# onesamblack/distributed-torch-horovod-gcp

Measured on NVIDIA H100. Metric: images/sec (whole job, device-timed, max over ranks) ResNet-50 synthetic ImageNet training, higher is better.
Workload: dtype bf16

## Files before the change

### distributed_torch_horovod_gcp_b200/csrc/conv_sm90.cu

```cuda
#include <cuda.h>
#include <cuda_bf16.h>
#include <cuda_runtime.h>
#include <limits.h>
#include <stdint.h>
#include <stdio.h>
#include <stdlib.h>
#include <string.h>

#include "sm90_common.cuh"

namespace {

constexpr int MAX_TAPS = 9;
constexpr int MAX_CLASSES = 4;

struct ConvTap {
  int amap;
  int dw, dh;
  int wcol;
};
struct ConvClass {
  int ntaps;
  int out_map;
  ConvTap taps[MAX_TAPS];
// ... 61 lines not shown
          } else {
#pragma unroll
            for (int c = 0; c < BN / 64; ++c)
              tma_load_2d(&maps.b, s.bar, s.b + c * (BLOCK_K * 128), tap.wcol + n_idx + 64 * c, kc * BLOCK_K);
          }
        }
      }
    } else {
      const int tile = w % tiles, split = w / tiles;
      const ConvTap tap = p.cls[0].taps[tile % p.num_taps_total];
      const int mn = tile / p.num_taps_total;
      const int m_idx = (mn / nnb) * BLOCK_M;
      const int n_idx = (mn % nnb) * BN;
      const int kb0 = split * kb_per_split;
      const int kb1 = min(kb0 + kb_per_split, pix_tiles);
      for (int kb = kb0; kb < kb1; ++kb) {
        const int w0 = (kb % p.tiles_w) * p.bw;
        const int h0 = ((kb / p.tiles_w) % p.tiles_h) * p.bh;
        const int n0 = (kb / (p.tiles_w * p.tiles_h)) * p.bn;
        const Stage s = next();
#pragma unroll
        for (int c = 0; c < BLOCK_M / 64; ++c)
          tma_load_4d(&maps.out[0], s.bar, s.a + c * (BLOCK_K * 128), m_idx + 64 * c, w0, h0, n0);
#pragma unroll
        for (int c = 0; c < BN / 64; ++c)
          tma_load_4d(&maps.a[tap.amap], s.bar, s.b + c * (BLOCK_K * 128), n_idx + 64 * c, w0 + tap.dw,
                      h0 + tap.dh, n0);
      }
    }
  }
  __device__ Slab slab(int w, int q) const {
    if (MODE != MODE_WGRAD) {
      const int nt = w % nnb;
      const int rest = w / nnb;
      const int mt = rest % pix_tiles;
      const int r0 = q * 32;
      StoreAt at;
      at.rank4 = 1;
      at.w = (mt % p.tiles_w) * p.bw + (r0 % p.bw);
      at.h = ((mt / p.tiles_w) % p.tiles_h) * p.bh + (r0 / p.bw) % p.bh;
      at.n = (mt / (p.tiles_w * p.tiles_h)) * p.bn + r0 / (p.bw * p.bh);
      at.sw = p.sw; at.sh = p.sh;
      at.vw = p.out_w - at.w; at.vh = p.out_h - at.h; at.vn = p.out_n - at.n;
      return Slab{&maps.out[p.cls[rest / pix_tiles].out_map], 0, nt * BN, at, 0, 0, 0, 0};
    }
    const int tile = w % tiles;
    const ConvTap tap = p.cls[0].taps[tile % p.num_taps_total];
    const int mn = tile / p.num_taps_total;
    const int m_idx = (mn / nnb) * BLOCK_M;
    return Slab{nullptr, m_idx + q * 32, (mn % nnb) * BN, StoreAt{}, tile, m_idx, tap.wcol, w / tiles};
  }
};

template <int BN, int MODE>
__global__ void __launch_bounds__(NUM_THREADS, 1)
conv_bf16_kernel(const __grid_constant__ ConvMaps maps, const __grid_constant__ ConvParams p) {
  persistent_body<BN, MODE == MODE_WGRAD, MODE != MODE_FPROP>(ConvWork<BN, MODE>(maps, p), p.g);
}

int make_map4(CUtensorMap* m, const void* ptr, uint64_t C, uint64_t Wd, uint64_t Hd, uint64_t Nd, uint64_t pw,
              uint64_t ph, uint64_t pn, uint32_t bw, uint32_t bh, uint32_t bn) {
  const cuuint64_t dims[4] = {C, Wd, Hd, Nd};
  const cuuint64_t strides[3] = {pw * 2, ph * 2, pn * 2};
  const cuuint32_t box[4] = {64, bw, bh, bn};
  return encode_map(m, ptr, 4, dims, strides, box);
}

void choose_box(int W, int H, int N, int rows, int* bw, int* bh, int* bn) {
  double best = 1e30;
  *bw = 1; *bh = 1; *bn = rows;
  for (int w = 1; w <= rows; w <<= 1) {
    for (int h = 1; w * h <= rows; h <<= 1) {
      const int n = rows / (w * h);
      const double covered = (double)((W + w - 1) / w * w) * ((H + h - 1) / h * h) * ((N + n - 1) / n * n);
      const double score = covered - 1e-3 * w - 1e-6 * h;
      if (score < best) { best = score; *bw = w; *bh = h; *bn = n; }
    }
  }
}

int floordiv2(int e) { return (e >= 0) ? e / 2 : -((-e + 1) / 2); }

struct ConvShape {
  int N, H, W, Cin, Cout, R, S, stride, pad, OH, OW;
};

int check_shape(ConvShape& s) {
  if (s.R != s.S || (s.R != 1 && s.R != 3)) return fail("only 1x1 and 3x3 filters");
  if (s.pad != (s.R - 1) / 2) return fail("padding must be (R-1)/2");
  if (s.stride != 1 && s.stride != 2) return fail("stride must be 1 or 2");
  if (s.stride == 2 && ((s.H | s.W) & 1)) return fail("stride 2 needs even H and W");
  if ((s.Cin % 8) || (s.Cout % 8)) return fail("channels must be multiples of 8");
  s.OH = s.H / s.stride;
  s.OW = s.W / s.stride;
  return 0;
}

int make_parity_maps(CUtensorMap* maps, const void* base, int C, int W, int H, int N, int bw, int bh, int bn) {
  for (int ph = 0; ph < 2; ++ph)
    for (int pw = 0; pw < 2; ++pw) {
      const __nv_bfloat16* ptr = reinterpret_cast<const __nv_bfloat16*>(base) + ((size_t)ph * W + pw) * C;
      if (make_map4(&maps[ph * 2 + pw], ptr, C, W / 2, H / 2, N, 2 * (uint64_t)C, 2 * (uint64_t)W * C,
                    (uint64_t)H * W * C, bw, bh, bn))
        return -1;
    }
  return 0;
}

void forward_taps(ConvClass& cl, int R, int S, int Cin, int stride, int pad) {
  for (int r = 0; r < R; ++r)
    for (int c = 0; c < S; ++c) {
      ConvTap& t = cl.taps[cl.ntaps++];
      const int eh = r - pad, ew = c - pad;
      if (stride == 1) {
        t.amap = 0; t.dh = eh; t.dw = ew;
      } else {
        const int ph = eh & 1, pw = ew & 1;
        t.amap = ph * 2 + pw; t.dh = floordiv2(eh - ph); t.dw = floordiv2(ew - pw);
      }
      t.wcol = (r * S + c) * Cin;
    }
}

void slab_box(ConvParams& p) {
  p.sw = p.bw < 32 ? p.bw : 32;
  p.sh = (32 / p.sw) < p.bh ? (32 / p.sw) : p.bh;
}

template <int MODE>
int launch_conv(const ConvMaps& maps, const ConvParams& p, int BN, int work, int max_ctas, cudaStream_t st) {
  if (BN == 64) return launch_persistent<conv_bf16_kernel<64, MODE>, 64>(work, max_ctas, st, maps, p);
  return launch_persistent<conv_bf16_kernel<128, MODE>, 128>(work, max_ctas, st, maps, p);
}

ConvParams conv_params() {
  ConvParams p;
  memset(&p, 0, sizeof(p));
  p.g.M = INT_MAX;
  p.g.splits = 1;
  p.g.alpha = 1.0f;
  return p;
}

}

extern "C" {

const char* b200dp_conv_last_error() { return g_err; }

int b200dp_conv_fprop(const void* x, const void* w, void* y, int N, int H, int W, int Cin, int Cout, int R, int S,
                      int stride, int pad, int block_n, int max_ctas, float* stats, unsigned long long stream) {
  if (ensure_init()) return -1;
  ConvShape s{N, H, W, Cin, Cout, R, S, stride, pad, 0, 0};
  if (check_shape(s)) return -1;
  if (((uintptr_t)x | (uintptr_t)w | (uintptr_t)y) & 15) return fail("pointers must be 16-byte aligned");
  const int BN = pick_bn(Cout, block_n);
  if (BN < 0) return -1;
  ConvMaps maps;
  ConvParams p = conv_params();
  p.g.N = Cout; p.g.ldc = Cout; p.g.C = y; p.g.out_mode = 0;
  p.g.stats = stats;
  if (stats != nullptr && Cout > STATS_MAX_N) return fail("stats: Cout <= 2048 required");
  p.g.num_n_blocks = (Cout + BN - 1) / BN;
  p.g.num_k_blocks = (Cin + BLOCK_K - 1) / BLOCK_K;
  p.kc_per_tap = p.g.num_k_blocks;
  choose_box(s.OW, s.OH, N, BLOCK_M, &p.bw, &p.bh, &p.bn);
  p.tiles_w = (s.OW + p.bw - 1) / p.bw; p.tiles_h = (s.OH + p.bh - 1) / p.bh; p.tiles_n = (N + p.bn - 1) / p.bn;
  p.num_classes = 1;
  p.num_taps_total = R * S;
  p.out_w = s.OW; p.out_h = s.OH; p.out_n = N;
  forward_taps(p.cls[0], R, S, Cin, stride, pad);
  if (stride == 1) {
    if (make_map4(&maps.a[0], x, Cin, W, H, N, Cin, (uint64_t)W * Cin, (uint64_t)H * W * Cin, p.bw, p.bh, p.bn))
      return -1;
    maps.a[1] = maps.a[2] = maps.a[3] = maps.a[0];
  } else if (make_parity_maps(maps.a, x, Cin, W, H, N, p.bw, p.bh, p.bn)) {
    return -1;
  }
  if (make_map2(&maps.b, w, Cout, (uint64_t)R * S * Cin, (uint64_t)R * S * Cin, BN)) return -1;
  slab_box(p);
  if (make_map4(&maps.out[0], y, Cout, s.OW, s.OH, N, Cout, (uint64_t)s.OW * Cout, (uint64_t)s.OH * s.OW * Cout, p.sw,
                p.sh, 32 / (p.sw * p.sh)))
    return -1;
  maps.out[1] = maps.out[2] = maps.out[3] = maps.out[0];
  const int work = p.tiles_w * p.tiles_h * p.tiles_n * p.g.num_n_blocks;
// ... 119 lines not shown
```

### distributed_torch_horovod_gcp_b200/csrc/gemm_sm90.cu

```cuda
#include <cuda.h>
#include <cuda_bf16.h>
#include <cuda_runtime.h>
#include <stdint.h>

#include "sm90_common.cuh"

namespace {

template <int BN, bool A_MN, bool B_MN>
struct GemmWork {
  static constexpr bool kStats = true, kSplitK = true;
  const CUtensorMap *a, *b, *c;
  const GemmParams& p;
  int tiles, items, kb_per_split;

  __device__ GemmWork(const CUtensorMap* a_, const CUtensorMap* b_, const CUtensorMap* c_, const GemmParams& p_)
      : a(a_), b(b_), c(c_), p(p_), tiles(p_.num_m_blocks * p_.num_n_blocks), items(tiles * p_.splits),
        kb_per_split((p_.num_k_blocks + p_.splits - 1) / p_.splits) {}
  __device__ void prefetch() const {
    tma_prefetch_desc(a);
    tma_prefetch_desc(b);
    if (p.out_mode == 0) tma_prefetch_desc(c);
  }
  __device__ int m_idx(int tile) const {
    return (p.n_fastest ? tile / p.num_n_blocks : tile % p.num_m_blocks) * BLOCK_M;
  }
  __device__ int n_idx(int tile) const { return (p.n_fastest ? tile % p.num_n_blocks : tile / p.num_m_blocks) * BN; }
  __device__ int num_kb(int w) const {
    const int kb0 = (w / tiles) * kb_per_split;
    return min(kb0 + kb_per_split, p.num_k_blocks) - kb0;
  }
  template <class Next>
  __device__ void load(int w, Next& next) const {
    const int tile = w % tiles;
    const int m0 = m_idx(tile), n0 = n_idx(tile);
    const int kb0 = (w / tiles) * kb_per_split;
    const int kb1 = min(kb0 + kb_per_split, p.num_k_blocks);
    for (int kb = kb0; kb < kb1; ++kb) {
      const Stage s = next();
      const int k_idx = kb * BLOCK_K;
      if (!A_MN) {
        tma_load_2d(a, s.bar, s.a, k_idx, m0);
      } else {
#pragma unroll
        for (int c = 0; c < BLOCK_M / 64; ++c)
          tma_load_2d(a, s.bar, s.a + c * (BLOCK_K * 128), m0 + 64 * c, k_idx);
      }
      if (!B_MN) {
        tma_load_2d(b, s.bar, s.b, k_idx, n0);
      } else {
#pragma unroll
        for (int c = 0; c < BN / 64; ++c)
          tma_load_2d(b, s.bar, s.b + c * (BLOCK_K * 128), n0 + 64 * c, k_idx);
      }
    }
  }
  __device__ Slab slab(int w, int q) const {
    const int tile = w % tiles, split = w / tiles;
    const int m0 = m_idx(tile);
    return Slab{c, m0 + q * 32, n_idx(tile), StoreAt{}, tile, m0, 0, split};
  }
};

template <int BN, bool A_MN, bool B_MN>
__global__ void __launch_bounds__(NUM_THREADS, 1)
gemm_bf16_kernel(const __grid_constant__ CUtensorMap map_a, const __grid_constant__ CUtensorMap map_b,
                 const __grid_constant__ CUtensorMap map_c, const __grid_constant__ GemmParams p) {
  persistent_body<BN, A_MN, B_MN>(GemmWork<BN, A_MN, B_MN>(&map_a, &map_b, &map_c, p), p);
}

int launch_bn(int BN, int a_mn, int b_mn, const CUtensorMap& ma, const CUtensorMap& mb, const CUtensorMap& mc,
              const GemmParams& p, int max_ctas, cudaStream_t st) {
  const int work = p.num_m_blocks * p.num_n_blocks * p.splits;
#define LAUNCH(BNV, AMN, BMN) \
  launch_persistent<gemm_bf16_kernel<BNV, AMN, BMN>, BNV>(work, max_ctas, st, ma, mb, mc, p)
#define DISPATCH(BNV)                                          \
  if (BN == BNV) {                                             \
    if (!a_mn && !b_mn) return LAUNCH(BNV, false, false);      \
    if (!a_mn && b_mn) return LAUNCH(BNV, false, true);        \
    if (a_mn && !b_mn) return LAUNCH(BNV, true, false);        \
    return LAUNCH(BNV, true, true);                            \
  }
  DISPATCH(64)
  DISPATCH(128)
#undef DISPATCH
#undef LAUNCH
  return fail("unreachable");
}

}

extern "C" {

const char* b200dp_gemm_last_error() { return g_err; }

int b200dp_gemm_bf16(const void* A, const void* B, void* C, int M, int N, int K, int lda, int ldb, int ldc,
                     int a_mn, int b_mn, const void* bias_bf16, const void* bias_f32, const void* residual,
                     void* preact, int act, int out_mode, int out_bf16, float alpha, int splits, int block_n,
                     int max_ctas, float* stats, const void* res_mask, unsigned long long stream) {
  if (ensure_init()) return -1;
  if (M <= 0 || N <= 0 || K <= 0) return fail("bad shape");
  if ((N % 8) || (lda % 8) || (ldb % 8) || (ldc % 4) || ((out_mode == 0 || out_bf16) && (ldc % 8)))
    return fail("alignment: N, lda, ldb, ldc must be multiples of 8");
  if (((uintptr_t)A | (uintptr_t)B | (uintptr_t)C) & 15) return fail("pointers must be 16-byte aligned");
  const int BN = pick_bn(N, block_n);
  if (BN < 0) return -1;
  GemmParams p{};
  p.M = M; p.N = N; p.ldc = ldc;
  p.num_m_blocks = (M + BLOCK_M - 1) / BLOCK_M;
  p.num_n_blocks = (N + BN - 1) / BN;
  p.num_k_blocks = (K + BLOCK_K - 1) / BLOCK_K;
  p.splits = normalize_splits(splits, p.num_k_blocks);
  if (p.splits > 1 && (out_mode == 0 || bias_bf16 || bias_f32 || residual || preact || act))
    return fail("split-K requires out_mode 1/2 without bias, residual or activation");
  p.act = act; p.out_mode = out_mode; p.c_bf16 = out_bf16 ? 1 : 0; p.C = C; p.bias = bias_bf16; p.bias_f32 = bias_f32;
  p.residual = residual; p.preact = preact; p.alpha = alpha;
  p.stats = stats;
  p.res_mask = reinterpret_cast<const unsigned char*>(res_mask);
  if (res_mask != nullptr && (residual == nullptr || preact != nullptr || act > 2 || out_mode != 0 || (N % 64) ||
                              ldc != N))
    return fail("res_mask: plain bf16 residual, dense rows and N % 64 == 0 required");
  if (stats != nullptr && (N > STATS_MAX_N || out_mode != 0)) return fail("stats: N <= 2048 and bf16 output required");
  p.n_fastest = ((size_t)N * (size_t)K * 2 <= ((size_t)20 << 20)) ? 1 : 0;
  CUtensorMap ma, mb, mc;
  if (a_mn ? make_map2(&ma, A, K, M, lda, BLOCK_K) : make_map2(&ma, A, M, K, lda, BLOCK_M)) return -1;
  if (b_mn ? make_map2(&mb, B, K, N, ldb, BLOCK_K) : make_map2(&mb, B, N, K, ldb, BN)) return -1;
  if (out_mode == 0) {
    if (make_map2(&mc, C, M, N, ldc, 32)) return -1;
  } else {
    mc = ma;
  }
  cudaStream_t st = (cudaStream_t)(uintptr_t)stream;
  if (p.splits > 1) p.splitk_slice = (long long)M * ldc;
  return run_splitk(p, p.num_m_blocks * p.num_n_blocks, st,
                    [&] { return launch_bn(BN, a_mn, b_mn, ma, mb, mc, p, max_ctas, st); });
}

}
```

### distributed_torch_horovod_gcp_b200/csrc/sm90_common.cuh

```cuda
#pragma once
#include <cuda.h>
#include <cuda_bf16.h>
#include <cuda_runtime.h>
#include <stdint.h>
#include <stdio.h>

namespace {

constexpr int BLOCK_M = 128;
constexpr int BLOCK_K = 64;
constexpr int WGMMA_K = 16;
constexpr int NUM_THREADS = 384;
constexpr int SMEM_LIMIT = 232448;

struct GemmParams {
  int M, N;
  int ldc;
  int num_m_blocks, num_n_blocks, num_k_blocks;
  int splits;
  int act;
  int out_mode;
  int c_bf16;
  void* C;
  const void* bias;
  const void* bias_f32;
  const void* residual;
  void* preact;
  int n_fastest;
  float alpha;
  const unsigned char* res_mask;
  float* stats;
  float* splitk_ws;
  int* splitk_count;
  long long splitk_slice;
};

constexpr int STATS_MAX_N = 2048;
constexpr int STATS_WARP_FLOATS = 256;
constexpr int STATS_SMEM_BYTES = 8 * STATS_WARP_FLOATS * 4;

__device__ __forceinline__ uint32_t smem_u32(const void* p) {
  return static_cast<uint32_t>(__cvta_generic_to_shared(p));
}
__device__ __forceinline__ void mbar_init(uint64_t* bar, uint32_t count) {
  asm volatile("mbarrier.init.shared::cta.b64 [%0], %1;" ::"r"(smem_u32(bar)), "r"(count));
}
__device__ __forceinline__ void mbar_expect_tx(uint64_t* bar, uint32_t bytes) {
  asm volatile("mbarrier.arrive.expect_tx.shared::cta.b64 _, [%0], %1;" ::"r"(smem_u32(bar)),
               "r"(bytes)
               : "memory");
}
__device__ __forceinline__ void mbar_arrive(uint64_t* bar) {
  asm volatile("mbarrier.arrive.shared::cta.b64 _, [%0];" ::"r"(smem_u32(bar)) : "memory");
}
__device__ __forceinline__ void mbar_wait(uint64_t* bar, uint32_t parity) {
  uint32_t done = 0;
  unsigned long long t0 = 0;
  for (uint32_t tries = 0; !done; ++tries) {
// ... 15 lines not shown
  }
}
__device__ __forceinline__ void tma_load_2d(const CUtensorMap* map, uint64_t* bar, void* dst, int c0,
                                            int c1) {
  asm volatile(
      "cp.async.bulk.tensor.2d.shared::cluster.global.mbarrier::complete_tx::bytes [%0], [%1, {%3, %4}], "
      "[%2];" ::"r"(smem_u32(dst)),
      "l"(map), "r"(smem_u32(bar)), "r"(c0), "r"(c1)
      : "memory");
}
__device__ __forceinline__ void tma_store_2d(const CUtensorMap* map, const void* src, int c0, int c1) {
  asm volatile("cp.async.bulk.tensor.2d.global.shared::cta.bulk_group [%0, {%2, %3}], [%1];" ::"l"(map),
               "r"(smem_u32(src)), "r"(c0), "r"(c1)
               : "memory");
}
__device__ __forceinline__ void tma_load_4d(const CUtensorMap* map, uint64_t* bar, void* dst, int c0, int c1,
                                            int c2, int c3) {
  asm volatile(
      "cp.async.bulk.tensor.4d.shared::cluster.global.mbarrier::complete_tx::bytes [%0], "
      "[%1, {%3, %4, %5, %6}], [%2];" ::"r"(smem_u32(dst)),
      "l"(map), "r"(smem_u32(bar)), "r"(c0), "r"(c1), "r"(c2), "r"(c3)
      : "memory");
}
__device__ __forceinline__ void tma_store_4d(const CUtensorMap* map, const void* src, int c0, int c1, int c2,
                                             int c3) {
  asm volatile("cp.async.bulk.tensor.4d.global.shared::cta.bulk_group [%0, {%2, %3, %4, %5}], [%1];" ::"l"(map),
               "r"(smem_u32(src)), "r"(c0), "r"(c1), "r"(c2), "r"(c3)
               : "memory");
}
__device__ __forceinline__ void tma_store_commit() { asm volatile("cp.async.bulk.commit_group;" ::: "memory"); }
template <int N>
__device__ __forceinline__ void tma_store_wait_read() {
  asm volatile("cp.async.bulk.wait_group.read %0;" ::"n"(N) : "memory");
}
__device__ __forceinline__ void tma_store_wait_all() { asm volatile("cp.async.bulk.wait_group 0;" ::: "memory"); }
__device__ __forceinline__ void fence_async_smem() { asm volatile("fence.proxy.async.shared::cta;" ::: "memory"); }
__device__ __forceinline__ void tma_prefetch_desc(const CUtensorMap* map) {
  asm volatile("prefetch.tensormap [%0];" ::"l"(map) : "memory");
}
__device__ __forceinline__ void wg_fence() { asm volatile("wgmma.fence.sync.aligned;" ::: "memory"); }
__device__ __forceinline__ void wg_commit() { asm volatile("wgmma.commit_group.sync.aligned;" ::: "memory"); }
template <int N>
__device__ __forceinline__ void wg_wait() {
  asm volatile("wgmma.wait_group.sync.aligned %0;" ::"n"(N) : "memory");
}
template <int R>
__device__ __forceinline__ void wg_fence_operands(float* d) {
#pragma unroll
  for (int i = 0; i < R; ++i) asm volatile("" : "+f"(d[i])::"memory");
}
__device__ __forceinline__ void named_bar(int id, int count) {
  asm volatile("bar.sync %0, %1;" ::"r"(id), "r"(count) : "memory");
}

template <int TA, int TB>
__device__ __forceinline__ void wgmma_bf16_n64(float* d, uint64_t a, uint64_t b, uint32_t acc) {
  asm volatile(
      "{\n\t.reg .pred p;\n\tsetp.ne.b32 p, %34, 0;\n\t"
      "wgmma.mma_async.sync.aligned.m64n64k16.f32.bf16.bf16 {%0, %1, %2, %3, %4, %5, %6, %7, %8, %9, %10, %11, %12, %13, %14, %15, %16, %17, %18, %19, %20, %21, %22, %23, %24, %25, %26, %27, %28, %29, %30, %31}, %32, %33, p, 1, 1, %35, %36;\n\t}\n"
      : "+f"(d[0]), "+f"(d[1]), "+f"(d[2]), "+f"(d[3]), "+f"(d[4]), "+f"(d[5]), "+f"(d[6]), "+f"(d[7]), "+f"(d[8]), "+f"(d[9]), "+f"(d[10]), "+f"(d[11]), "+f"(d[12]), "+f"(d[13]), "+f"(d[14]), "+f"(d[15]), "+f"(d[16]), "+f"(d[17]), "+f"(d[18]), "+f"(d[19]), "+f"(d[20]), "+f"(d[21]), "+f"(d[22]), "+f"(d[23]), "+f"(d[24]), "+f"(d[25]), "+f"(d[26]), "+f"(d[27]), "+f"(d[28]), "+f"(d[29]), "+f"(d[30]), "+f"(d[31])
      : "l"(a), "l"(b), "r"(acc), "n"(TA), "n"(TB));
}

template <int TA, int TB>
__device__ __forceinline__ void wgmma_bf16_n128(float* d, uint64_t a, uint64_t b, uint32_t acc) {
  asm volatile(
      "{\n\t.reg .pred p;\n\tsetp.ne.b32 p, %66, 0;\n\t"
      "wgmma.mma_async.sync.aligned.m64n128k16.f32.bf16.bf16 {%0, %1, %2, %3, %4, %5, %6, %7, %8, %9, %10, %11, %12, %13, %14, %15, %16, %17, %18, %19, %20, %21, %22, %23, %24, %25, %26, %27, %28, %29, %30, %31, %32, %33, %34, %35, %36, %37, %38, %39, %40, %41, %42, %43, %44, %45, %46, %47, %48, %49, %50, %51, %52, %53, %54, %55, %56, %57, %58, %59, %60, %61, %62, %63}, %64, %65, p, 1, 1, %67, %68;\n\t}\n"
      : "+f"(d[0]), "+f"(d[1]), "+f"(d[2]), "+f"(d[3]), "+f"(d[4]), "+f"(d[5]), "+f"(d[6]), "+f"(d[7]), "+f"(d[8]), "+f"(d[9]), "+f"(d[10]), "+f"(d[11]), "+f"(d[12]), "+f"(d[13]), "+f"(d[14]), "+f"(d[15]), "+f"(d[16]), "+f"(d[17]), "+f"(d[18]), "+f"(d[19]), "+f"(d[20]), "+f"(d[21]), "+f"(d[22]), "+f"(d[23]), "+f"(d[24]), "+f"(d[25]), "+f"(d[26]), "+f"(d[27]), "+f"(d[28]), "+f"(d[29]), "+f"(d[30]), "+f"(d[31]), "+f"(d[32]), "+f"(d[33]), "+f"(d[34]), "+f"(d[35]), "+f"(d[36]), "+f"(d[37]), "+f"(d[38]), "+f"(d[39]), "+f"(d[40]), "+f"(d[41]), "+f"(d[42]), "+f"(d[43]), "+f"(d[44]), "+f"(d[45]), "+f"(d[46]), "+f"(d[47]), "+f"(d[48]), "+f"(d[49]), "+f"(d[50]), "+f"(d[51]), "+f"(d[52]), "+f"(d[53]), "+f"(d[54]), "+f"(d[55]), "+f"(d[56]), "+f"(d[57]), "+f"(d[58]), "+f"(d[59]), "+f"(d[60]), "+f"(d[61]), "+f"(d[62]), "+f"(d[63])
      : "l"(a), "l"(b), "r"(acc), "n"(TA), "n"(TB));
}

__device__ __forceinline__ void wgmma_tf32_n32(float* d, uint64_t a, uint64_t b, uint32_t acc) {
  asm volatile(
      "{\n\t.reg .pred p;\n\tsetp.ne.b32 p, %18, 0;\n\t"
      "wgmma.mma_async.sync.aligned.m64n32k8.f32.tf32.tf32 {%0, %1, %2, %3, %4, %5, %6, %7, %8, %9, %10, %11, %12, %13, %14, %15}, %16, %17, p, 1, 1;\n\t}\n"
      : "+f"(d[0]), "+f"(d[1]), "+f"(d[2]), "+f"(d[3]), "+f"(d[4]), "+f"(d[5]), "+f"(d[6]), "+f"(d[7]), "+f"(d[8]), "+f"(d[9]), "+f"(d[10]), "+f"(d[11]), "+f"(d[12]), "+f"(d[13]), "+f"(d[14]), "+f"(d[15])
      : "l"(a), "l"(b), "r"(acc));
}


__device__ __forceinline__ uint64_t make_desc(uint32_t smem_addr, uint32_t lbo_bytes,
                                              uint32_t sbo_bytes) {
  uint64_t d = 0;
  d |= (uint64_t)((smem_addr & 0x3FFFF) >> 4);
  d |= (uint64_t)((lbo_bytes >> 4) & 0x3FFF) << 16;
  d |= (uint64_t)((sbo_bytes >> 4) & 0x3FFF) << 32;
  d |= (uint64_t)1 << 62;
  return d;
}

__device__ __forceinline__ bool elect_one() {
  uint32_t pred;
  asm volatile(
      "{\n\t"
      ".reg .pred p;\n\t"
      "elect.sync _|p, 0xffffffff;\n\t"
      "selp.u32 %0, 1, 0, p;\n\t"
      "}\n"
      : "=r"(pred));
  return pred != 0;
}

__device__ __forceinline__ uint64_t make_desc_base(uint32_t lbo_bytes, uint32_t sbo_bytes) {
  return make_desc(0, lbo_bytes, sbo_bytes);
}
__device__ __forceinline__ uint64_t desc_addr(uint32_t smem_addr) { return (uint64_t)((smem_addr & 0x3FFFF) >> 4); }

template <int BN, bool TA, bool TB>
__device__ __forceinline__ void wgmma_bf16(float* d, uint64_t a, uint64_t b, uint32_t acc) {
  static_assert(BN == 64 || BN == 128, "wgmma width");
  if constexpr (BN == 64) wgmma_bf16_n64<TA ? 1 : 0, TB ? 1 : 0>(d, a, b, acc);
  else wgmma_bf16_n128<TA ? 1 : 0, TB ? 1 : 0>(d, a, b, acc);
}

template <int BN, bool A_MN, bool B_MN, int STAGES, int A_BYTES, int B_BYTES>
__device__ __forceinline__ void wg_mainloop(float* d, uint32_t sa, uint32_t sb, uint64_t* full_bar, uint64_t* empty_bar,
                                            int& stage, uint32_t& phase, int nkb, int wg) {
  constexpr uint32_t KSTEP_A = A_MN ? ((WGMMA_K * 128) >> 4) : ((WGMMA_K * 2) >> 4);
  constexpr uint32_t KSTEP_B = B_MN ? ((WGMMA_K * 128) >> 4) : ((WGMMA_K * 2) >> 4);
  const uint64_t a0 = (A_MN ? make_desc_base(BLOCK_K * 128, 1024) : make_desc_base(16, 1024)) +
                      desc_addr(sa + (uint32_t)wg * 8192u);
  const uint64_t b0 = (B_MN ? make_desc_base(BLOCK_K * 128, 1024) : make_desc_base(16, 1024)) + desc_addr(sb);
  const bool leader = (threadIdx.x & 127) == 0;
  int prev = -1;
  for (int kb = 0; kb < nkb; ++kb) {
    mbar_wait(&full_bar[stage], phase);
    const uint64_t da = a0 + (uint64_t)(stage * (A_BYTES >> 4));
    const uint64_t db = b0 + (uint64_t)(stage * (B_BYTES >> 4));
    wg_fence();
#pragma unroll
    for (int k = 0; k < BLOCK_K / WGMMA_K; ++k)
      wgmma_bf16<BN, A_MN, B_MN>(d, da + k * KSTEP_A, db + k * KSTEP_B, (kb | k) ? 1u : 0u);
    wg_commit();
    wg_wait<1>();
    if (prev >= 0 && leader) mbar_arrive(&empty_bar[prev]);
    prev = stage;
    if (++stage == STAGES) { stage = 0; phase ^= 1; }
  }
  wg_wait<0>();
  wg_fence_operands<BN / 2>(d);
  if (prev >= 0 && leader) mbar_arrive(&empty_bar[prev]);
}

__device__ __forceinline__ float fast_erf(float x) {
  const float ax = fabsf(x);
  const float t = __fdividef(1.0f, fmaf(0.3275911f, ax, 1.0f));
  float poly = fmaf(1.061405429f, t, -1.453152027f);
  poly = fmaf(poly, t, 1.421413741f);
  poly = fmaf(poly, t, -0.284496736f);
  poly = fmaf(poly, t, 0.254829592f);
  const float y = 1.0f - poly * t * __expf(-ax * ax);
  return copysignf(y, x);
}
__device__ __forceinline__ float gelu_erf(float x) {
  return 0.5f * x * (1.0f + fast_erf(x * 0.70710678118654752f));
}

__device__ __forceinline__ float gelu_erf_grad(float x) {
  const float cdf = 0.5f * (1.0f + fast_erf(x * 0.70710678118654752f));
  const float pdf = 0.3989422804014327f * __expf(-0.5f * x * x);
  return cdf + x * pdf;
}

__device__ __forceinline__ void unpack8(const uint4& x, float* f) {
  const uint32_t wv[4] = {x.x, x.y, x.z, x.w};
#pragma unroll
  for (int t = 0; t < 4; ++t) {
    f[2 * t] = __uint_as_float(wv[t] << 16);
    f[2 * t + 1] = __uint_as_float(wv[t] & 0xffff0000u);
  }
}

template <int BN>
struct Cfg {
  static constexpr int A_BYTES = BLOCK_M * BLOCK_K * 2;
  static constexpr int B_BYTES = BN * BLOCK_K * 2;
  static constexpr int STAGE_BYTES = A_BYTES + B_BYTES;
  static constexpr int NCH = BN / 64;
  static constexpr int STORE_BYTES = BLOCK_M * BN * 2;
  static constexpr int FIXED_BYTES = STORE_BYTES + 1024  + 256  + STATS_SMEM_BYTES;
  static constexpr int STAGES = (SMEM_LIMIT - FIXED_BYTES) / STAGE_BYTES;
  static constexpr int SMEM_BYTES = STAGES * STAGE_BYTES + FIXED_BYTES;
  static_assert(STAGES >= 4, "shared memory");
  static_assert(2 * STAGES * 8 <= 256, "barrier space");
};

struct StoreAt {
  int rank4, w, h, n;
  int sw, sh, vw, vh, vn;
};

__device__ __forceinline__ void epi_sts128(uint32_t addr, const uint4& v) {
  asm volatile("st.shared.v4.b32 [%0], {%1, %2, %3, %4};" ::"r"(addr), "r"(v.x), "r"(v.y), "r"(v.z), "r"(v.w) : "memory");
}
__device__ __forceinline__ void epi_sts32(uint32_t addr, uint32_t v) {
  asm volatile("st.shared.b32 [%0], %1;" ::"r"(addr), "r"(v) : "memory");
}
__device__ __forceinline__ uint32_t epi_lds32(uint32_t addr) {
  uint32_t v;
  asm volatile("ld.shared.b32 %0, [%1];" : "=r"(v) : "r"(addr) : "memory");
  return v;
}
__device__ __forceinline__ uint32_t prmt_sign(uint32_t a, uint32_t sel) {
  uint32_t d;
  asm("prmt.b32 %0, %1, %2, %3;" : "=r"(d) : "r"(a), "r"(0u), "r"(sel));
  return d;
}
__device__ __forceinline__ uint32_t cvt_bf16x2(float lo, float hi) {
  uint32_t o;
  asm("cvt.rn.bf16x2.f32 %0, %1, %2;" : "=r"(o) : "f"(hi), "f"(lo));
  return o;
}
__device__ __forceinline__ float zero_plus_ftz(float v) {
  float o;
  asm("add.ftz.f32 %0, %1, %2;" : "=f"(o) : "f"(0.0f), "f"(v));
  return o;
}

template <int BN>
__device__ __forceinline__ uint32_t stage_off(int r, int u) {
  return (uint32_t)((((r >> 5) * (BN / 64) + (u >> 3)) << 12) + ((r & 31) << 7) + (((u ^ r) & 7) << 4));
}

template <int BN>
__device__ __forceinline__ void res_load(const GemmParams& p, uint4* rv, int m0, int r0, int n_idx, int lane) {
  const __nv_bfloat16* rbase = reinterpret_cast<const __nv_bfloat16*>(p.residual);
#pragma unroll
  for (int i = 0; i < BN / 16; ++i) {
    const int e = i * 32 + lane, row = m0 + r0 + e / (BN / 8), col = n_idx + (e % (BN / 8)) * 8;
    rv[i] = (row < p.M && col < p.N) ? *reinterpret_cast<const uint4*>(rbase + (size_t)row * p.ldc + col)
                                     : make_uint4(0, 0, 0, 0);
  }
  if (p.res_mask != nullptr) {
// ... 97 lines not shown
          v1 = fmaxf(v1, 0.0f);
        } else if (p.act == 2) {
          v0 = gelu_erf(v0);
          v1 = gelu_erf(v1);
        }
        if (p.residual != nullptr) {
          const uint32_t a = epi_lds32(sa(j, h));
          const float a0 = __uint_as_float(a << 16), a1 = __uint_as_float(a & 0xffff0000u);
          if (p.act == 3) {
            v0 *= gelu_erf_grad(a0);
            v1 *= gelu_erf_grad(a1);
          } else if (p.act == 4) {
            v0 = a0 > 0.0f ? v0 : 0.0f;
            v1 = a1 > 0.0f ? v1 : 0.0f;
          } else {
            v0 += a0;
            v1 += a1;
          }
        }
      }
      if (p.out_mode == 0) {
        epi_sts32(sa(j, h), cvt_bf16x2(v0, v1));
      } else if (row < p.M && col_ok) {
        const size_t e = (size_t)row * p.ldc + col;
        if (p.splits > 1) {
          float* dst = reinterpret_cast<float*>(cbase) + e;
          asm volatile("st.global.v2.f32 [%0], {%1, %2};" ::"l"(dst), "f"(v0), "f"(v1) : "memory");
        } else {
          v0 = zero_plus_ftz(v0);
          v1 = zero_plus_ftz(v1);
          if (p.c_bf16) {
            __nv_bfloat16* dst = reinterpret_cast<__nv_bfloat16*>(cbase) + e;
            if (p.out_mode == 1) {
              uint32_t o;
              asm volatile("ld.global.b32 %0, [%1];" : "=r"(o) : "l"(dst) : "memory");
              v0 += __uint_as_float(o << 16);
              v1 += __uint_as_float(o & 0xffff0000u);
            }
            asm volatile("st.global.b32 [%0], %1;" ::"l"(dst), "r"(cvt_bf16x2(v0, v1)) : "memory");
          } else {
            float* dst = reinterpret_cast<float*>(cbase) + e;
            if (p.out_mode == 2)
              asm volatile("st.global.v2.f32 [%0], {%1, %2};" ::"l"(dst), "f"(v0), "f"(v1) : "memory");
            else
              asm volatile("red.global.add.v2.f32 [%0], {%1, %2};" ::"l"(dst), "f"(v0), "f"(v1) : "memory");
          }
        }
      }
    }
  }
}

template <int BN>
__device__ __forceinline__ void store_slab(const GemmParams& p, const CUtensorMap* map_c, const uint8_t* stg_ptr,
                                           int q, int lane, int m_row0, int n_idx, int c_begin, int c_end,
                                           const StoreAt at, float* s_stats) {
#pragma unroll 1
  for (int c0 = c_begin; c0 < c_end; c0 += 64) {
    const int col0 = n_idx + c0;
    if (col0 >= p.N) continue;
    const uint8_t* buf = stg_ptr + ((q * (BN / 64) + (c0 >> 6)) << 12);
    if (s_stats != nullptr) {
      float sum_lo = 0.f, sum_hi = 0.f, sq_lo = 0.f, sq_hi = 0.f;
      const uint32_t base = smem_u32(buf) + (uint32_t)((lane & 3) << 2);
      const uint32_t u = (uint32_t)(lane >> 2);
      if (at.rank4 || m_row0 + 32 > p.M) {
        bool ok;
        if (at.rank4) {
          const int rw = lane % at.sw, rh = (lane / at.sw) % at.sh, rn = lane / (at.sw * at.sh);
          ok = rw < at.vw && rh < at.vh && rn < at.vn;
        } else {
          ok = m_row0 + lane < p.M;
        }
        const uint32_t rows_ok = __ballot_sync(0xffffffffu, ok);
#pragma unroll
        for (int rr = 0; rr < 32; ++rr) {
          uint32_t w = epi_lds32(base + rr * 128 + ((u ^ (rr & 7)) << 4));
          if (!((rows_ok >> rr) & 1u)) w = 0u;
          const float lo = __uint_as_float(w << 16), hi = __uint_as_float(w & 0xffff0000u);
          sum_lo += lo; sum_hi += hi;
          sq_lo = fmaf(lo, lo, sq_lo); sq_hi = fmaf(hi, hi, sq_hi);
        }
      } else {
#pragma unroll
        for (int rr = 0; rr < 32; ++rr) {
          const uint32_t w = epi_lds32(base + rr * 128 + ((u ^ (rr & 7)) << 4));
          const float lo = __uint_as_float(w << 16), hi = __uint_as_float(w & 0xffff0000u);
          sum_lo += lo; sum_hi += hi;
          sq_lo = fmaf(lo, lo, sq_lo); sq_hi = fmaf(hi, hi, sq_hi);
        }
      }
      const uint32_t ps = smem_u32(s_stats) + (uint32_t)(((c0 - c_begin) + 2 * lane) << 2);
      float a0, a1, b0, b1;
      asm volatile("ld.shared.v2.f32 {%0, %1}, [%2];" : "=f"(a0), "=f"(a1) : "r"(ps));
      asm volatile("ld.shared.v2.f32 {%0, %1}, [%2];" : "=f"(b0), "=f"(b1) : "r"(ps + (STATS_WARP_FLOATS / 2) * 4));
      asm volatile("st.shared.v2.f32 [%0], {%1, %2};" ::"r"(ps), "f"(a0 + sum_lo), "f"(a1 + sum_hi) : "memory");
      asm volatile("st.shared.v2.f32 [%0], {%1, %2};" ::"r"(ps + (STATS_WARP_FLOATS / 2) * 4), "f"(b0 + sq_lo),
                   "f"(b1 + sq_hi)
                   : "memory");
    }
    if (lane == 0) {
      if (at.rank4) tma_store_4d(map_c, buf, col0, at.w, at.h, at.n);
      else tma_store_2d(map_c, buf, col0, m_row0);
      tma_store_commit();
    }
  }
// ... 153 lines not shown
    }
  } else {
    asm volatile("setmaxnreg.inc.sync.aligned.u32 232;" ::: "memory");
    const int cw = warp - 4;
    const int wg = cw >> 2;
    const int r0 = wg * 64 + (cw & 3) * 16;
    const int q = cw & 3;
    const int half = cw >> 2;
    const int c_begin = (BN >= 128) ? half * (BN / 2) : 0;
    const int c_end = (BN >= 128) ? c_begin + BN / 2 : (half == 0 ? BN : 0);
    const int epi_tid = cw * 32 + lane;
    float* my_stats = s_stats + cw * STATS_WARP_FLOATS;
    const uint32_t stg = smem_u32(smem_store);
    __shared__ int s_last;
    int stats_n = -1;
    int stage = 0;
    uint32_t phase = 0;
    float d[BN / 2];
    for (int w = blockIdx.x; w < wk.items; w += gridDim.x) {
      const Slab s = wk.slab(w, q);
      wg_mainloop<BN, A_MN, B_MN, C::STAGES, C::A_BYTES, C::B_BYTES>(d, smem_u32(smem_a), smem_u32(smem_b), full_bar,
                                                                     empty_bar, stage, phase, wk.num_kb(w), wg);
      if (want_stats && s.n_idx != stats_n) {
        if (stats_n >= 0) stats_flush<BN>(p, s_stats, stats_n, epi_tid);
        stats_n = s.n_idx;
      }
      const bool res = p.residual != nullptr && p.out_mode != 1;
      uint4 rv[BN / 16];
      if (res) res_load<BN>(p, rv, s.m_idx, r0, s.n_idx, lane);
      if (p.out_mode == 0) {
        if (lane == 0) tma_store_wait_read<0>();
        named_bar(1, 256);
      }
      if (res) {
        __syncwarp();
        res_stage<BN>(rv, stg, r0, lane);
        __syncwarp();
      }
      epilogue_frag<BN>(p, d, stg, wg, s.m_idx, s.n_idx, s.split, s.c_off);
      if (p.out_mode == 0) {
        fence_async_smem();
        named_bar(1, 256);
        store_slab<BN>(p, s.map_c, smem_store, q, lane, s.m_row0, s.n_idx, c_begin, c_end, s.at,
                       want_stats ? my_stats : nullptr);
      }
      if (Work::kSplitK && p.splits > 1) splitk_finish_tile(p, s.tile, s.m_idx, s.n_idx, BN, s.c_off, epi_tid, &s_last);
    }
    if (want_stats && stats_n >= 0) stats_flush<BN>(p, s_stats, stats_n, epi_tid);
    if (want_stats) stats_finalize(p, epi_tid);
    if (p.out_mode == 0 && lane == 0) tma_store_wait_all();
  }
}

typedef CUresult (*EncodeTiledFn)(CUtensorMap*, CUtensorMapDataType, cuuint32_t, void*, const cuuint64_t*,
                                  const cuuint64_t*, const cuuint32_t*, const cuuint32_t*,
                                  CUtensorMapInterleave, CUtensorMapSwizzle, CUtensorMapL2promotion,
                                  CUtensorMapFloatOOBfill);
EncodeTiledFn g_encode = nullptr;
thread_local char g_err[512];
int g_num_sms = 0;

int fail(const char* msg, int code = 0) {
  snprintf(g_err, sizeof(g_err), "%s (%d)", msg, code);
  return -1;
}

inline void bind_primary_context() {
  static thread_local bool bound = false;
  if (!bound) {
    cudaFree(nullptr);
    bound = true;
  }
}

int ensure_init() {
  bind_primary_context();
  if (g_encode) return 0;
  void* fn = nullptr;
  cudaDriverEntryPointQueryResult st;
  cudaError_t e = cudaGetDriverEntryPoint("cuTensorMapEncodeTiled", &fn, cudaEnableDefault, &st);
  if (e != cudaSuccess || st != cudaDriverEntryPointSuccess || !fn)
    return fail("cuTensorMapEncodeTiled entry point unavailable", (int)e);
  g_encode = reinterpret_cast<EncodeTiledFn>(fn);
  int dev = 0;
  cudaGetDevice(&dev);
  cudaDeviceGetAttribute(&g_num_sms, cudaDevAttrMultiProcessorCount, dev);
  return 0;
}

int encode_map(CUtensorMap* m, const void* ptr, int rank, const cuuint64_t* dims, const cuuint64_t* byte_strides,
               const cuuint32_t* box) {
  const cuuint32_t estr[4] = {1, 1, 1, 1};
  CUresult r = g_encode(m, CU_TENSOR_MAP_DATA_TYPE_BFLOAT16, rank, const_cast<void*>(ptr), dims, byte_strides, box,
                        estr, CU_TENSOR_MAP_INTERLEAVE_NONE, CU_TENSOR_MAP_SWIZZLE_128B,
                        CU_TENSOR_MAP_L2_PROMOTION_L2_256B, CU_TENSOR_MAP_FLOAT_OOB_FILL_NONE);
  if (r != CUDA_SUCCESS) return fail("cuTensorMapEncodeTiled failed", (int)r);
  return 0;
}

int make_map2(CUtensorMap* m, const void* ptr, uint64_t rows, uint64_t cols, uint64_t ld, uint32_t box_rows) {
  const cuuint64_t dims[2] = {cols, rows};
  const cuuint64_t strides[1] = {ld * 2};
  const cuuint32_t box[2] = {64, box_rows};
  return encode_map(m, ptr, 2, dims, strides, box);
}

template <auto Kernel>
int smem_attr_once(int bytes) {
  static bool attr_set = false;
  if (!attr_set) {
    cudaError_t e = cudaFuncSetAttribute(Kernel, cudaFuncAttributeMaxDynamicSharedMemorySize, bytes);
    if (e != cudaSuccess) return fail(cudaGetErrorString(e), (int)e);
    attr_set = true;
  }
  return 0;
}

template <auto Kernel, int BN, class... Args>
int launch_persistent(int work, int max_ctas, cudaStream_t st, const Args&... args) {
  if (smem_attr_once<Kernel>(Cfg<BN>::SMEM_BYTES)) return -1;
  int grid = work < g_num_sms ? work : g_num_sms;
  if (max_ctas > 0 && grid > max_ctas) grid = max_ctas;
  if (grid > STATS_MAX_CTAS) grid = STATS_MAX_CTAS;
  Kernel<<<grid, NUM_THREADS, Cfg<BN>::SMEM_BYTES, st>>>(args...);
  cudaError_t e = cudaGetLastError();
  if (e != cudaSuccess) return fail(cudaGetErrorString(e), (int)e);
  return 0;
}

template <class Launch>
int run_splitk(GemmParams& p, int tiles, cudaStream_t st, Launch&& launch) {
  void* ws = nullptr;
  if (p.splits > 1) {
    const size_t slices = (size_t)p.splits * (size_t)p.splitk_slice * sizeof(float);
    cudaError_t e = cudaMallocAsync(&ws, slices + (size_t)tiles * sizeof(int), st);
    if (e == cudaSuccess) {
      p.splitk_ws = reinterpret_cast<float*>(ws);
      p.splitk_count = reinterpret_cast<int*>(reinterpret_cast<char*>(ws) + slices);
      e = cudaMemsetAsync(p.splitk_count, 0, (size_t)tiles * sizeof(int), st);
    }
    if (e != cudaSuccess) return fail(cudaGetErrorString(e), (int)e);
  }
  const int rc = launch();
  if (ws != nullptr) {
    cudaError_t e = cudaFreeAsync(ws, st);
    if (e != cudaSuccess && rc == 0) return fail(cudaGetErrorString(e), (int)e);
  }
  return rc;
}

int normalize_splits(int splits, int kblocks) {
  if (splits > kblocks) splits = kblocks;
  if (splits < 1) splits = 1;
  const int per = (kblocks + splits - 1) / splits;
  return (kblocks + per - 1) / per;
}

int pick_bn(int n, int block_n) {
  if (block_n == 0) return n > 64 ? 128 : 64;
  if (block_n == 256) return 128;
  if (block_n != 64 && block_n != 128) return fail("block_n must be 64/128/256");
  return block_n;
}

}
```

Before: 5768.

## Add ping-pong warpgroup kernel body for BN=64 dgrad and plain GEMMs

Adds a ping-pong persistent body where the two consumer warpgroups alternate whole tiles. Each warpgroup computes a 128x64 tile with two accumulators and hands the tensor cores to the other warpgroup via named barriers, so one tile's epilogue overlaps the next tile's mainloop. It is used for BN=64 dgrad convolutions and for BN=64 GEMMs without a fused epilogue (no stats, bias or activation). Each warpgroup gets its own store buffer, which uses more shared memory and leaves fewer pipeline stages. The extra barrier coordination and phase-skipping logic add correctness risk.

```diff
diff --git a/distributed_torch_horovod_gcp_b200/csrc/conv_sm90.cu b/distributed_torch_horovod_gcp_b200/csrc/conv_sm90.cu
--- a/distributed_torch_horovod_gcp_b200/csrc/conv_sm90.cu
+++ b/distributed_torch_horovod_gcp_b200/csrc/conv_sm90.cu
@@ -137,10 +137,11 @@
   }
 };
 
-template <int BN, int MODE>
+template <int BN, int MODE, bool PP = MODE == MODE_DGRAD && BN == 64>
 __global__ void __launch_bounds__(NUM_THREADS, 1)
 conv_bf16_kernel(const __grid_constant__ ConvMaps maps, const __grid_constant__ ConvParams p) {
-  persistent_body<BN, MODE == MODE_WGRAD, MODE != MODE_FPROP>(ConvWork<BN, MODE>(maps, p), p.g);
+  if constexpr (PP) pingpong_body<BN, MODE == MODE_WGRAD, MODE != MODE_FPROP>(ConvWork<BN, MODE>(maps, p), p.g);
+  else persistent_body<BN, MODE == MODE_WGRAD, MODE != MODE_FPROP>(ConvWork<BN, MODE>(maps, p), p.g);
 }
 
 int make_map4(CUtensorMap* m, const void* ptr, uint64_t C, uint64_t Wd, uint64_t Hd, uint64_t Nd, uint64_t pw,
@@ -214,8 +215,12 @@
 
 template <int MODE>
 int launch_conv(const ConvMaps& maps, const ConvParams& p, int BN, int work, int max_ctas, cudaStream_t st) {
-  if (BN == 64) return launch_persistent<conv_bf16_kernel<64, MODE>, 64>(work, max_ctas, st, maps, p);
-  return launch_persistent<conv_bf16_kernel<128, MODE>, 128>(work, max_ctas, st, maps, p);
+  if constexpr (MODE == MODE_DGRAD) {
+    if (BN == 64 && !g_sm90_reference_body)
+      return launch_persistent<conv_bf16_kernel<64, MODE, true>, 64, true>(work, max_ctas, st, maps, p);
+  }
+  if (BN == 64) return launch_persistent<conv_bf16_kernel<64, MODE, false>, 64>(work, max_ctas, st, maps, p);
+  return launch_persistent<conv_bf16_kernel<128, MODE, false>, 128>(work, max_ctas, st, maps, p);
 }
 
 ConvParams conv_params() {
diff --git a/distributed_torch_horovod_gcp_b200/csrc/gemm_sm90.cu b/distributed_torch_horovod_gcp_b200/csrc/gemm_sm90.cu
--- a/distributed_torch_horovod_gcp_b200/csrc/gemm_sm90.cu
+++ b/distributed_torch_horovod_gcp_b200/csrc/gemm_sm90.cu
@@ -62,18 +62,29 @@
   }
 };
 
-template <int BN, bool A_MN, bool B_MN>
+template <int BN, bool A_MN, bool B_MN, bool PP>
 __global__ void __launch_bounds__(NUM_THREADS, 1)
 gemm_bf16_kernel(const __grid_constant__ CUtensorMap map_a, const __grid_constant__ CUtensorMap map_b,
                  const __grid_constant__ CUtensorMap map_c, const __grid_constant__ GemmParams p) {
-  persistent_body<BN, A_MN, B_MN>(GemmWork<BN, A_MN, B_MN>(&map_a, &map_b, &map_c, p), p);
+  if constexpr (PP) pingpong_body<BN, A_MN, B_MN>(GemmWork<BN, A_MN, B_MN>(&map_a, &map_b, &map_c, p), p);
+  else persistent_body<BN, A_MN, B_MN>(GemmWork<BN, A_MN, B_MN>(&map_a, &map_b, &map_c, p), p);
+}
+
+template <int BN, bool A_MN, bool B_MN>
+int launch_body(int work, const CUtensorMap& ma, const CUtensorMap& mb, const CUtensorMap& mc, const GemmParams& p,
+                int max_ctas, cudaStream_t st) {
+  if constexpr (BN == 64 && !A_MN && B_MN) {
+    if (p.stats == nullptr && p.out_mode == 0 && p.alpha == 1.0f && p.bias == nullptr && p.bias_f32 == nullptr &&
+        p.preact == nullptr && p.act == 0 && !g_sm90_reference_body)
+      return launch_persistent<gemm_bf16_kernel<BN, A_MN, B_MN, true>, BN, true>(work, max_ctas, st, ma, mb, mc, p);
+  }
+  return launch_persistent<gemm_bf16_kernel<BN, A_MN, B_MN, false>, BN>(work, max_ctas, st, ma, mb, mc, p);
 }
 
 int launch_bn(int BN, int a_mn, int b_mn, const CUtensorMap& ma, const CUtensorMap& mb, const CUtensorMap& mc,
               const GemmParams& p, int max_ctas, cudaStream_t st) {
   const int work = p.num_m_blocks * p.num_n_blocks * p.splits;
-#define LAUNCH(BNV, AMN, BMN) \
-  launch_persistent<gemm_bf16_kernel<BNV, AMN, BMN>, BNV>(work, max_ctas, st, ma, mb, mc, p)
+#define LAUNCH(BNV, AMN, BMN) launch_body<BNV, AMN, BMN>(work, ma, mb, mc, p, max_ctas, st)
 #define DISPATCH(BNV)                                          \
   if (BN == BNV) {                                             \
     if (!a_mn && !b_mn) return LAUNCH(BNV, false, false);      \
@@ -90,9 +101,13 @@
 
 }
 
+int g_sm90_reference_body = 0;
+
 extern "C" {
 
 const char* b200dp_gemm_last_error() { return g_err; }
+
+void b200dp_sm90_reference_body(int on) { g_sm90_reference_body = on; }
 
 int b200dp_gemm_bf16(const void* A, const void* B, void* C, int M, int N, int K, int lda, int ldb, int ldc,
                      int a_mn, int b_mn, const void* bias_bf16, const void* bias_f32, const void* residual,
diff --git a/distributed_torch_horovod_gcp_b200/csrc/sm90_common.cuh b/distributed_torch_horovod_gcp_b200/csrc/sm90_common.cuh
--- a/distributed_torch_horovod_gcp_b200/csrc/sm90_common.cuh
+++ b/distributed_torch_horovod_gcp_b200/csrc/sm90_common.cuh
@@ -4,6 +4,8 @@
 #include <cuda_runtime.h>
 #include <stdint.h>
 #include <stdio.h>
+
+extern int g_sm90_reference_body;
 
 namespace {
 
@@ -125,6 +127,9 @@
 __device__ __forceinline__ void named_bar(int id, int count) {
   asm volatile("bar.sync %0, %1;" ::"r"(id), "r"(count) : "memory");
 }
+__device__ __forceinline__ void named_bar_arrive(int id, int count) {
+  asm volatile("bar.arrive %0, %1;" ::"r"(id), "r"(count) : "memory");
+}
 
 template <int TA, int TB>
 __device__ __forceinline__ void wgmma_bf16_n64(float* d, uint64_t a, uint64_t b, uint32_t acc) {
@@ -216,6 +221,39 @@
   if (prev >= 0 && leader) mbar_arrive(&empty_bar[prev]);
 }
 
+template <int BN, bool A_MN, bool B_MN, int STAGES, int A_BYTES, int B_BYTES, class Issued>
+__device__ __forceinline__ void wg_mainloop_pp(float* d0, float* d1, uint32_t sa, uint32_t sb, uint64_t* full_bar,
+                                               uint64_t* empty_bar, int& stage, uint32_t& phase, int nkb,
+                                               Issued&& issued) {
+  constexpr uint32_t KSTEP_A = A_MN ? ((WGMMA_K * 128) >> 4) : ((WGMMA_K * 2) >> 4);
+  constexpr uint32_t KSTEP_B = B_MN ? ((WGMMA_K * 128) >> 4) : ((WGMMA_K * 2) >> 4);
+  const uint64_t a0 = (A_MN ? make_desc_base(BLOCK_K * 128, 1024) : make_desc_base(16, 1024)) + desc_addr(sa);
+  const uint64_t b0 = (B_MN ? make_desc_base(BLOCK_K * 128, 1024) : make_desc_base(16, 1024)) + desc_addr(sb);
+  const bool leader = (threadIdx.x & 127) == 0;
+  int prev = -1;
+  for (int kb = 0; kb < nkb; ++kb) {
+    mbar_wait(&full_bar[stage], phase);
+    const uint64_t da = a0 + (uint64_t)(stage * (A_BYTES >> 4));
+    const uint64_t db = b0 + (uint64_t)(stage * (B_BYTES >> 4));
+    wg_fence();
+#pragma unroll
+    for (int k = 0; k < BLOCK_K / WGMMA_K; ++k) {
+      wgmma_bf16<BN, A_MN, B_MN>(d0, da + k * KSTEP_A, db + k * KSTEP_B, (kb | k) ? 1u : 0u);
+      wgmma_bf16<BN, A_MN, B_MN>(d1, da + (8192 >> 4) + k * KSTEP_A, db + k * KSTEP_B, (kb | k) ? 1u : 0u);
+    }
+    wg_commit();
+    wg_wait<1>();
+    if (prev >= 0 && leader) mbar_arrive(&empty_bar[prev]);
+    prev = stage;
+    if (++stage == STAGES) { stage = 0; phase ^= 1; }
+  }
+  issued();
+  wg_wait<0>();
+  wg_fence_operands<BN / 2>(d0);
+  wg_fence_operands<BN / 2>(d1);
+  if (prev >= 0 && leader) mbar_arrive(&empty_bar[prev]);
+}
+
 __device__ __forceinline__ float fast_erf(float x) {
   const float ax = fabsf(x);
   const float t = __fdividef(1.0f, fmaf(0.3275911f, ax, 1.0f));
@@ -245,14 +283,15 @@
   }
 }
 
-template <int BN>
+template <int BN, bool PP = false>
 struct Cfg {
   static constexpr int A_BYTES = BLOCK_M * BLOCK_K * 2;
   static constexpr int B_BYTES = BN * BLOCK_K * 2;
   static constexpr int STAGE_BYTES = A_BYTES + B_BYTES;
   static constexpr int NCH = BN / 64;
   static constexpr int STORE_BYTES = BLOCK_M * BN * 2;
-  static constexpr int FIXED_BYTES = STORE_BYTES + 1024  + 256  + STATS_SMEM_BYTES;
+  static constexpr int FIXED_BYTES =
+      (PP ? 2 : 1) * STORE_BYTES + 1024  + 256  + (PP ? 0 : STATS_SMEM_BYTES);
   static constexpr int STAGES = (SMEM_LIMIT - FIXED_BYTES) / STAGE_BYTES;
   static constexpr int SMEM_BYTES = STAGES * STAGE_BYTES + FIXED_BYTES;
   static_assert(STAGES >= 4, "shared memory");
@@ -456,6 +495,33 @@
 }
 
 template <int BN>
+__device__ __forceinline__ void epilogue_plain(const float* d, uint32_t stg, int wg, bool res) {
+  const int t = threadIdx.x & 127, lane = t & 31;
+  const int r = wg * 64 + (t >> 5) * 16 + (lane >> 2);
+  const uint32_t x = (uint32_t)(r & 7);
+  const uint32_t sbase = stg + (uint32_t)(((r >> 5) * (BN / 64)) << 12) + (uint32_t)((r & 31) << 7) +
+                         (uint32_t)(lane & 3) * 4u;
+  auto sa = [&](int j, int h) -> uint32_t {
+    return sbase + (uint32_t)(h * 1024 + ((j >> 3) << 12)) + ((((uint32_t)j & 7u) ^ x) << 4);
+  };
+  if (!res) {
+#pragma unroll
+    for (int j = 0; j < BN / 8; ++j)
+#pragma unroll
+      for (int h = 0; h < 2; ++h) epi_sts32(sa(j, h), cvt_bf16x2(d[4 * j + 2 * h], d[4 * j + 2 * h + 1]));
+    return;
+  }
+#pragma unroll
+  for (int j = 0; j < BN / 8; ++j)
+#pragma unroll
+    for (int h = 0; h < 2; ++h) {
+      const uint32_t a = epi_lds32(sa(j, h));
+      epi_sts32(sa(j, h), cvt_bf16x2(d[4 * j + 2 * h] + __uint_as_float(a << 16),
+                                     d[4 * j + 2 * h + 1] + __uint_as_float(a & 0xffff0000u)));
+    }
+}
+
+template <int BN>
 __device__ __forceinline__ void store_slab(const GemmParams& p, const CUtensorMap* map_c, const uint8_t* stg_ptr,
                                            int q, int lane, int m_row0, int n_idx, int c_begin, int c_end,
                                            const StoreAt at, float* s_stats) {
@@ -715,6 +781,93 @@
   }
 }
 
+template <int BN, bool A_MN, bool B_MN, class Work>
+__device__ __forceinline__ void pingpong_body(const Work& wk, const GemmParams& p) {
+  static_assert(BN == 64, "ping-pong tiles are 128 x 64");
+  using C = Cfg<BN, true>;
+  extern __shared__ __align__(1024) uint8_t smem_raw[];
+  uint8_t* smem = reinterpret_cast<uint8_t*>((reinterpret_cast<uintptr_t>(smem_raw) + 1023) &
+                                             ~static_cast<uintptr_t>(1023));
+  uint8_t* smem_a = smem;
+  uint8_t* smem_b = smem + C::STAGES * C::A_BYTES;
+  uint8_t* smem_store = smem + C::STAGES * C::STAGE_BYTES;
+  uint64_t* bars = reinterpret_cast<uint64_t*>(smem_store + 2 * C::STORE_BYTES);
+  uint64_t* full_bar = bars;
+  uint64_t* empty_bar = bars + C::STAGES;
+
+  const int warp = threadIdx.x >> 5;
+  const int lane = threadIdx.x & 31;
+
+  if (warp == 0 && lane == 0) {
+    wk.prefetch();
+    for (int i = 0; i < C::STAGES; ++i) {
+      mbar_init(&full_bar[i], 1);
+      mbar_init(&empty_bar[i], 1);
+    }
+    asm volatile("fence.mbarrier_init.release.cluster;" ::: "memory");
+  }
+  __syncthreads();
+
+  if (warp < 4) {
+    asm volatile("setmaxnreg.dec.sync.aligned.u32 40;" ::: "memory");
+    if (warp == 0 && elect_one()) {
+      int stage = 0;
+      uint32_t phase = 0;
+      auto next = [&]() {
+        mbar_wait(&empty_bar[stage], phase ^ 1);
+        mbar_expect_tx(&full_bar[stage], C::STAGE_BYTES);
+        const Stage s{smem_a + stage * C::A_BYTES, smem_b + stage * C::B_BYTES, &full_bar[stage]};
+        if (++stage == C::STAGES) { stage = 0; phase ^= 1; }
+        return s;
+      };
+      for (int w = blockIdx.x; w < wk.items; w += gridDim.x) wk.load(w, next);
+    }
+  } else {
+    asm volatile("setmaxnreg.inc.sync.aligned.u32 232;" ::: "memory");
+    const int wg = (warp - 4) >> 2;
+    const int q = warp & 3;
+    uint8_t* const my_store = smem_store + wg * C::STORE_BYTES;
+    const uint32_t stg = smem_u32(my_store);
+    int stage = 0;
+    uint32_t phase = 0;
+    float d0[BN / 2], d1[BN / 2];
+    int i = 0;
+    for (int w = blockIdx.x; w < wk.items; w += gridDim.x, ++i) {
+      if ((i & 1) != wg) {
+        const int n = stage + wk.num_kb(w);
+        if ((n / C::STAGES) & 1) phase ^= 1;
+        stage = n % C::STAGES;
+        continue;
+      }
+      const Slab s = wk.slab(w, q);
+      if (i > 0) named_bar(3 + wg, 256);
+      const bool pass = w + (int)gridDim.x < wk.items;
+      wg_mainloop_pp<BN, A_MN, B_MN, C::STAGES, C::A_BYTES, C::B_BYTES>(
+          d0, d1, smem_u32(smem_a), smem_u32(smem_b), full_bar, empty_bar, stage, phase, wk.num_kb(w),
+          [&] { if (pass) named_bar_arrive(4 - wg, 256); });
+      const bool res = p.residual != nullptr;
+      if (lane == 0) tma_store_wait_read<0>();
+      named_bar(1 + wg, 128);
+      if (res) {
+#pragma unroll
+        for (int h = 0; h < 2; ++h) {
+          uint4 rv[BN / 16];
+          res_load<BN>(p, rv, s.m_idx, h * 64 + q * 16, s.n_idx, lane);
+          __syncwarp();
+          res_stage<BN>(rv, stg, h * 64 + q * 16, lane);
+        }
+        __syncwarp();
+      }
+      epilogue_plain<BN>(d0, stg, 0, res);
+      epilogue_plain<BN>(d1, stg, 1, res);
+      fence_async_smem();
+      named_bar(1 + wg, 128);
+      store_slab<BN>(p, s.map_c, my_store, q, lane, s.m_row0, s.n_idx, 0, BN, s.at, nullptr);
+    }
+    if (lane == 0) tma_store_wait_all();
+  }
+}
+
 typedef CUresult (*EncodeTiledFn)(CUtensorMap*, CUtensorMapDataType, cuuint32_t, void*, const cuuint64_t*,
                                   const cuuint64_t*, const cuuint32_t*, const cuuint32_t*,
                                   CUtensorMapInterleave, CUtensorMapSwizzle, CUtensorMapL2promotion,
@@ -779,13 +932,13 @@
   return 0;
 }
 
-template <auto Kernel, int BN, class... Args>
+template <auto Kernel, int BN, bool PP = false, class... Args>
 int launch_persistent(int work, int max_ctas, cudaStream_t st, const Args&... args) {
-  if (smem_attr_once<Kernel>(Cfg<BN>::SMEM_BYTES)) return -1;
+  if (smem_attr_once<Kernel>(Cfg<BN, PP>::SMEM_BYTES)) return -1;
   int grid = work < g_num_sms ? work : g_num_sms;
   if (max_ctas > 0 && grid > max_ctas) grid = max_ctas;
   if (grid > STATS_MAX_CTAS) grid = STATS_MAX_CTAS;
-  Kernel<<<grid, NUM_THREADS, Cfg<BN>::SMEM_BYTES, st>>>(args...);
+  Kernel<<<grid, NUM_THREADS, Cfg<BN, PP>::SMEM_BYTES, st>>>(args...);
   cudaError_t e = cudaGetLastError();
   if (e != cudaSuccess) return fail(cudaGetErrorString(e), (int)e);
   return 0;
```

Result: no change. 5773, median of 6 (+0.1%).
